# cy-rae/fast-slam

Hardware: AMD Instinct MI355X
Metric: particle-updates/s (higher is better)
Workload: dtype f64

## Files before the change

fast-slam_amd/csrc/fs2_api.hip:

```cpp
#include <hip/hip_runtime.h>

#include <sched.h>
#include <unistd.h>

#include <algorithm>
#include <atomic>
#include <chrono>
#include <condition_variable>
#include <functional>
#include <cmath>
#include <cstdarg>
#include <cstdio>
#include <cstdlib>
#include <cstring>
#include <mutex>
#include <string>
#include <thread>
#include <tuple>
#include <vector>

#include "../../include/fs2.h"
#include "fs2_comm.hpp"
#include "fs2_frontend.hpp"
#include "fs2_kernels.hpp"
// ... 280 lines not shown
struct MtCtx {
    fs2_mt_state in;
    double sigma = 0.0;
    int64_t N = 0, P = 0, A = 0, amb_cap = 0, pos0 = 0, have = 0, total = 0;
    int h0 = 0;
    fs2_mt_state *after = nullptr, *after_u0 = nullptr;
    double *u0_out = nullptr;
};

struct fs2_handle {
    fs2_config cfg{};
    int64_t n_global = 0, n = 0, first = 0;
    hipStream_t stream = nullptr;
    int cur = 0;
    double *x[2] = {}, *y[2] = {}, *yaw[2] = {}, *w[2] = {};
    int32_t *cnt[2] = {};
    char *pool = nullptr;
    int64_t npool = 0;
    GrowMem pool_vm, rpool_vm;
    GrowMem mark_vm, freel_vm, rmark_vm, rfreel_vm;
    int64_t bcnt_cap = 0, rbcnt_cap = 0;
    Desc *pt[2] = {};
    uint32_t *bbox[2] = {};
    XDesc *rdesc = nullptr;
    XDesc *udesc = nullptr;
    size_t udesc_cap = 0;
    unsigned long long *xt_key = nullptr;
    uint32_t *xt_ref = nullptr, *xt_uidx = nullptr, *xt_cmask = nullptr, *xt_cbase = nullptr;
    uint32_t *xt_eslot = nullptr, *xt_ulist = nullptr;
    int64_t xt_cap = 0, xt_ecap = 0;
    SumFrame frame{-127.0f, 1.0f, 1.0f};
    float ext_seen = 0.0f;
    float *slb = nullptr;
    float *slb_pass = nullptr;
    uint32_t *ext_dev = nullptr;
    size_t rdesc_cap = 0;
    int rows = 0;
    uint32_t *freel = nullptr;
    int64_t nfree = 0, cursor = 0;
    uint8_t *mark = nullptr;
    uint32_t *sent_mask = nullptr;
    uint8_t epoch = 0;
    int64_t *bcnt = nullptr;
    int64_t *nfree_dev = nullptr;
    uint64_t collections = 0;
    char *rpool = nullptr;
// ... 137 lines not shown
    std::vector<uint8_t> imported;
    PeerMaps peers_host{};
    PeerMaps *peers_dev = nullptr;
    uint8_t *ep_dev = nullptr, *epochs_dev = nullptr;
    int64_t remote_rows = 0;
    int64_t remote_pages = INT64_MAX;
    int64_t remote_bound() const { return std::min(remote_rows, remote_pages); }
    int32_t collect_next = 0;
    ChainSummary *dch_send = nullptr, *dch_recv = nullptr;
    RankRecordX *recx = nullptr, *recxs = nullptr;
    double *est_base = nullptr;
    int32_t *uop = nullptr;
    NpTailPlan *np_tail_g = nullptr;
    std::vector<std::pair<hipEvent_t, hipEvent_t>> xev;
    size_t xev_used = 0;
    struct Guard {
        char *at;
        const char *name;
    };
    std::vector<Guard> guards;

    MapRef map() const {
        return MapRef{pool, pt[cur], std::max<int64_t>(n, 1), rows, rpool, frame, slb, row_boxes(cur),
                      refs_shared ? peers_dev : nullptr};
    }
    uint32_t *row_boxes(int b) const { return rows <= kBBoxRows ? bbox[b] : nullptr; }
    int64_t nblocks() const { return (n + kBlock - 1) / kBlock; }
    int reduce() const {
        const int mode = cfg.reduce_mode;
        if (tp) {
            if (mode == FS2_REDUCE_SEQUENTIAL) return FS2_REDUCE_SEQUENTIAL;
            return (mode != FS2_REDUCE_PARALLEL && xsh_ok) ? FS2_REDUCE_EXACT : FS2_REDUCE_PARALLEL;
        }
        if (mode != FS2_REDUCE_AUTO) return mode;
        return n_global <= 4096 ? FS2_REDUCE_SEQUENTIAL : FS2_REDUCE_EXACT;
    }
    ChainParams chain(const double *a, const double *bsum, double *c, double *total, bool lazy) const {
        ChainParams p{};
        p.a = a;
        p.n = n;
        p.bsum = bsum;
        p.nb = (int32_t)nblocks();
        p.lazy = lazy ? 1 : 0;
        p.uinfo = uinfo;
        p.udelta = udelta;
        p.ugl = ugl;
        p.uol = uol;
        p.bD = bD;
        p.bC = bC;
// ... 43 lines not shown
        if (bytes <= cap) continue;
        hipFree(p);
        p = nullptr;
        cap = 0;
        HIP_TRY(h, hipMalloc(&p, bytes));
        cap = bytes;
    }
    return FS2_OK;
}

static int reserve_xfer_table(fs2_handle *h, int64_t cap, int64_t nrows, bool in_scan);
static int xfer_bufs(fs2_handle *h) {
    const int64_t S = std::max<int64_t>(h->n, 1) * h->rows;
    int lg = 10;
    while ((int64_t(1) << lg) < 2 * S && lg < 31) ++lg;
    const int rc = reserve_xfer_table(h, int64_t(1) << lg, S, false);
    return rc ? rc : recv_bufs(h, sizeof(XDesc) * (size_t)S);
}

static int sync_sets(fs2_handle *h) {
    if (!h->sets_dev) return FS2_OK;
    BufSet b[2];
    for (int k = 0; k < 2; ++k)
        b[k] = BufSet{h->x[k], h->y[k], h->yaw[k], h->w[k], h->cnt[k], h->pt[k], h->row_boxes(k)};
    HIP_TRY(h, copy_sync(h, h->sets_dev, b, sizeof b, hipMemcpyHostToDevice));
    return FS2_OK;
}

static int grow_rows(fs2_handle *h, int need_slots) {
    if (need_slots <= h->cap) return FS2_OK;
    if (need_slots > h->max_cap)
        return set_err(&h->err, FS2_ERR_CAPACITY, "map needs %d landmark slots, limit is %d",
                       need_slots, h->max_cap);
    int rows = (need_slots + kPageSlots - 1) / kPageSlots;
    if (h->rows > 0) {
        const int geo = h->rows + std::max(h->rows / 4, 8);
        const int lim = std::min(h->max_cap / kPageSlots, rows <= kBBoxRows ? kBBoxRows : INT_MAX);
        rows = std::max(rows, std::min(geo, lim));
    }
    const size_t row_bytes = sizeof(Desc) * (size_t)std::max<int64_t>(h->n, 1);
    HIP_TRY(h, hipStreamSynchronize(h->stream));
    for (int b = 0; b < 2; ++b) {
        Desc *p = nullptr;
        HIP_TRY(h, hipMalloc(&p, row_bytes * rows));
        if (h->pt[b] && b == h->cur) HIP_TRY(h, copy_sync(h, p, h->pt[b], row_bytes * h->rows, hipMemcpyDeviceToDevice));
        hipFree(h->pt[b]);
        h->pt[b] = p;
    }
    h->rows = rows;
    h->cap = rows * kPageSlots;
    if (int rc = sync_sets(h)) return rc;
    if (h->rdesc) return xfer_bufs(h);
    return FS2_OK;
}

static int refs_short(fs2_handle *h, const char *what) {
    return set_err(&h->err, FS2_ERR_CAPACITY,
                   "page_refs mode: the %s pool ran short between collective collections (pools shared with "
                   "the other ranks cannot grow; size them with page_pool / record_pool)",
                   what);
}

static int collect_body(fs2_handle *h, bool records);
struct PoolTimer {
    fs2_handle *h;
    bool grow;
    std::chrono::steady_clock::time_point t0 = std::chrono::steady_clock::now();
    ~PoolTimer() {
        const double ms = std::chrono::duration<double, std::milli>(std::chrono::steady_clock::now() - t0).count();
        if (grow) {
// ... 790 lines not shown
    return g_last_error.c_str();
}

static void free_handle(fs2_handle *h) {
    if (!h) return;
    int prev_dev = -1;
    if (hipGetDevice(&prev_dev) != hipSuccess) prev_dev = -1;
    if (prev_dev != h->cfg.device) (void)hipSetDevice(h->cfg.device);
    if (h->stream) hipStreamSynchronize(h->stream);
    if (h->mt.dstream) hipStreamSynchronize(h->mt.dstream);
    const bool vmm = h->pool_vm.base || h->rpool_vm.base || h->freel_vm.base || h->mark_vm.base ||
                     h->rfreel_vm.base || h->rmark_vm.base;
    if (vmm) hipDeviceSynchronize();
    if (h->refs_shared && h->tp && !h->tp->in_process()) {
        std::string e;
        if (h->tp->allgather(h->ep_dev, h->epochs_dev, 1, h->stream, &e) == FS2_OK) hipStreamSynchronize(h->stream);
        h->tp->unshare();
        if (h->tp->allgather(h->ep_dev, h->epochs_dev, 1, h->stream, &e) == FS2_OK) hipStreamSynchronize(h->stream);
    }
    for (int s = 0; s < 2; ++s) {
        hipFree(h->x[s]); hipFree(h->y[s]); hipFree(h->yaw[s]); hipFree(h->w[s]); hipFree(h->cnt[s]);
        hipFree(h->pt[s]);
        hipFree(h->bbox[s]);
    }
    hipFree(h->rdesc); hipFree(h->udesc);
    hipFree(h->xt_key); hipFree(h->xt_ref); hipFree(h->xt_uidx); hipFree(h->xt_cmask); hipFree(h->xt_cbase);
    hipFree(h->xt_eslot); hipFree(h->xt_ulist);
    hipFree(h->sent_mask);
    if (h->pool_vm.base) gm_free(h->pool_vm);
    else hipFree(h->pool);
    if (h->rpool_vm.base) gm_free(h->rpool_vm);
    else hipFree(h->rpool);
    if (h->freel_vm.base) gm_free(h->freel_vm); else hipFree(h->freel);
    if (h->mark_vm.base) gm_free(h->mark_vm); else hipFree(h->mark);
    if (h->rfreel_vm.base) gm_free(h->rfreel_vm); else hipFree(h->rfreel);
    if (h->rmark_vm.base) gm_free(h->rmark_vm); else hipFree(h->rmark);
    if (vmm) hipDeviceSynchronize();
    hipFree(h->bcnt); hipFree(h->nfree_dev);
    hipFree(h->rbcnt); hipFree(h->rnfree_dev);
    hipFree(h->slb); hipFree(h->slb_pass); hipFree(h->ext_dev);
    hipFree(h->rank_d); hipFree(h->rank_e); hipFree(h->iblk);
    hipFree(h->mlo); hipFree(h->mhi); hipFree(h->out_src); hipFree(h->runs); hipFree(h->runs_n);
    hipFree(h->rec); hipFree(h->recs); hipFree(h->totals); hipFree(h->xrow); hipFree(h->xmat);
    hipFree(h->sarena);
    hipFree(h->rarena);
    hipFree(h->cand); hipFree(h->ncand);
// ... 355 lines not shown

static int fold_profile(fs2_handle *h) {
    const int used = h->ev.used;
    h->ev.used = 0;
    for (int k = 0; k < used; ++k) {
        const int rc = fold_one(h, k);
        if (rc) return rc;
    }
    return FS2_OK;
}

static int fold_one(fs2_handle *h, int set) {
    const ProfScan &p = h->ev.scan[set];
    hipEvent_t *E = h->ev.e[set];
    HIP_TRY(h, hipEventSynchronize(E[3]));
    const DevStats &st = p.st;
    float a = 0, f = 0, r = 0, x = 0, t = 0;
    HIP_TRY(h, hipEventElapsedTime(&a, E[0], E[2]));
    HIP_TRY(h, hipEventElapsedTime(&r, E[5], E[3]));
    HIP_TRY(h, hipEventElapsedTime(&t, E[0], E[3]));
    const uint64_t n = (uint64_t)h->n, nblk = (uint64_t)h->nblocks();
    const uint64_t box_rows = h->row_boxes(h->cur) ? (uint64_t)h->rows : 0ull;
    const bool filt = h->cfg.gate_filter != 0;
    const uint64_t cand_bytes = filt ? sizeof(Desc) * st.groups + 128ull * st.opened + 8ull * st.words +
                                           8ull * n * p.passes + 4ull * box_rows * nblk
                                     : 0ull;
    const uint64_t upd_fixed = p.fixed_bytes + (filt ? 4ull * n * p.passes : 0ull) + 8ull * n * (uint64_t)p.m;
    const uint64_t exact_bytes = upd_fixed + (filt ? 8ull * st.words : 0ull) + 48ull * st.candidates +
                                 (64ull + sizeof(Desc)) * st.written + (2ull * kPageBytes + sizeof(Desc)) * st.cow_pages +
                                 8ull * box_rows * nblk;
    if (filt && p.m <= kMaxM) {
        HIP_TRY(h, hipEventElapsedTime(&f, E[0], E[1]));
        HIP_TRY(h, hipEventElapsedTime(&x, E[4], E[2]));
        h->prof.exact_launches += 1;
        h->prof.exact_ms += x;
        h->prof.filter_launches += 1;
        h->prof.filter_ms += f;
        h->prof.filter_bytes += cand_bytes;
        h->prof.model_groups += st.groups;
        h->prof.model_opened += st.opened;
        h->prof.model_words += st.words;
        h->prof.model_candidates += st.candidates;
        h->prof.model_written += st.written;
        h->prof.model_cow += st.cow_pages;
        h->prof.model_fixed_bytes += upd_fixed;
        h->prof.model_box_bytes += 12ull * box_rows * nblk;
    }
    h->prof.scans += 1;
    h->prof.update_launches += p.passes;
    h->prof.update_ms += a;
    h->prof.reduce_ms += r;
    h->prof.scan_ms += t;
    h->prof.update_bytes += cand_bytes + exact_bytes;
    if (st.resampled)
        h->prof.resample_bytes += 2ull * sizeof(Desc) * (st.resample_slots / kPageSlots) +
                                  2ull * 36ull * (uint64_t)h->n + 40ull * (uint64_t)h->n;
    return FS2_OK;
}

static int wait_flag(fs2_handle *h, unsigned long long seq) {
    const auto t0 = std::chrono::steady_clock::now();
    for (unsigned it = 0;; ++it) {
        if (__atomic_load_n(h->pub_flag, __ATOMIC_ACQUIRE) == seq) return FS2_OK;
        if ((it & 1023u) == 1023u && std::chrono::steady_clock::now() - t0 > std::chrono::milliseconds(50)) break;
        __builtin_ia32_pause();
    }
    HIP_TRY(h, hipStreamSynchronize(h->stream));
    if (__atomic_load_n(h->pub_flag, __ATOMIC_ACQUIRE) != seq)
        return set_err(&h->err, FS2_ERR_HIP, "scan statistics were not published");
// ... 54 lines not shown

    const int nxt = 1 - cur;
    ResampleParams rs{};
    rs.n = h->n;
    rs.N = h->n_global;
    rs.a = h->first;
    rs.ao = h->first;
    rs.keep = h->shard;
    rs.ranges_mode = (sh && h->follow) ? 1 : 3;
    rs.w = h->w[cur];
    rs.c = h->cbuf;
    rs.bsum = h->bsum;
    rs.nblk = (int32_t)((h->n + 1023) / 1024);
    rs.mlo = h->mlo;
    rs.mhi = h->mhi;
    rs.out_src = h->out_src;
    rs.runs = h->runs;
    rs.runs_n = h->runs_n;
    rs.x = h->x[cur]; rs.y = h->y[cur]; rs.yaw = h->yaw[cur]; rs.cnt = h->cnt[cur];
    rs.ox = h->x[nxt]; rs.oy = h->y[nxt]; rs.oyaw = h->yaw[nxt]; rs.ow = h->w[nxt]; rs.ocnt = h->cnt[nxt];
    rs.map = h->map();
    rs.opt = h->pt[nxt];
    rs.obbox = h->row_boxes(nxt);
    rs.rank_d = h->rank_d;
    rs.rank_e = h->rank_e;
    rs.iblk = h->iblk;
    rs.part_best_w = h->part_best_w;
    rs.part_best_i = h->part_best_i;
    rs.part_slots = h->part_slots;
    rs.stats = h->stats_dev;
    rs.rec = h->rec;
    rs.flip_margin = flip_margin;
    rs.use_chain = exact ? 1 : 0;
    rs.refs = h->refs ? 1 : 0;
    if (h->refs && h->xt_key) {
        rs.tkey = h->xt_key;
        rs.tcap = h->xt_cap;
        rs.tepoch = ++h->loc_epoch;
    }
    rs.chain = ChainView{h->uinfo, h->ugl, h->uol, h->bpd, h->bpc, h->seql, h->sout, h->uel, h->bpe};
    rs.gen = sh ? nullptr : h->gen_dev;

    const bool xsh = sh && exact;
    if (prof && exact && !xsh && h->n <= 0) HIP_TRY(h, hipEventRecord(E[5], s));
    if (exact && !xsh) {
        ChainParams cp = h->chain(h->w[cur], h->wpart, nullptr, &h->stats_dev->total, false);
// ... 79 lines not shown
            HIP_TRY(h, launch_chain_fold(h->dch_recv, G, h->shard, h->rank_of, nullptr, &h->stats_dev->offset,
                                         h->stats_dev, s));
            cp.chain_first = h->shard == 0 ? 1 : 0;
            cp.force_list0 = 1;
            cp.s_entry = &h->stats_dev->offset;
            HIP_TRY(h, launch_chain_walk_from(cp, s));
        }
        if (!sh) {
            rs.est_early = 1;
            rs.go = h->go_dev;
            rs.go_seq = pseq;
        }
        HIP_TRY(h, launch_resample_ranges(rs, s, sh));
        if (!sh)
            HIP_TRY(h, launch_tail_single(rs, rp, h->pub_stats_dev, h->pub_flag_dev, pseq, s, nullptr));
        if (sh) {
            rc = exchange_particles(h, rs);
            if (rc) return rc;
            if (posted_stats(h).max_count > h->cap) scan_alloc(h, "scan_alloc rows (slots M)", (size_t)posted_stats(h).max_count << 20);
            rc = grow_rows(h, posted_stats(h).max_count);
            if (rc) return rc;
            rs.opt = h->pt[nxt];
            rs.obbox = h->row_boxes(nxt);
            rc = reserve_recs(h, h->u_recv * kPageSlots, &rs.alloc);
            if (rc) return rc;
            rc = reserve_pages(h, h->u_recv, &rs.alloc);
            if (rc) return rc;
            rs.map = h->map();
            const size_t rbytes = sizeof(XDesc) * (size_t)std::max<int64_t>((int64_t)h->n_recv * h->rows, 1);
            const size_t ubytes = sizeof(XDesc) * (size_t)std::max<int64_t>(h->u_recv, 1);
            if (rbytes > h->rdesc_cap || ubytes > h->udesc_cap) {
                scan_alloc(h, "scan_alloc recv rows (MiB)", std::max(rbytes, ubytes));
                rc = recv_bufs(h, std::max(rbytes, ubytes));
                if (rc) return rc;
            }
            rs.udesc = h->udesc;
            rs.rdesc = h->rdesc;
        }
        HIP_TRY(h, launch_resample_apply(rs, sh, s));
        if (sh) {
            {
                CommTimer ct(h);
                rc = h->tp->allgather(h->rec, h->recs, sizeof(RankRecord), s, &h->err);
            }
            if (rc) return rc;
            HIP_TRY(h, launch_global_best(rp, s));
// ... 1633 lines not shown
```

fast-slam_amd/csrc/fs2_kernels.hpp:

```cpp
#pragma once

#include <hip/hip_ext.h>
#include <hip/hip_runtime.h>
#include <stdint.h>

#include <vector>

namespace fs2 {

constexpr int kBlock = 256;
constexpr int kPageSlots = 8;
constexpr int kMaxSlots = 4096;
constexpr int kMaxRows = kMaxSlots / kPageSlots;
constexpr int kMaxM = 4;
constexpr int kScanGroup = kPageSlots;
constexpr int kMaxCand = 8;

constexpr int kPageBytes = 128;
constexpr int kRecBytes = 48;
constexpr uint32_t kOwned = 0x80000000u;
constexpr uint32_t kIdMask = 0x7fffffffu;
constexpr uint32_t kRecIdLimit = 0xffffffffu;
typedef uint32_t Desc;
typedef uint2 XDesc;

struct SumFrame {
    float org, cell;
    float icell;
};
constexpr uint32_t kSumOpen = 0xff00ff00u;

constexpr int kBBoxRows = 256;
constexpr uint32_t kBoxEmpty = 0x00ff00ffu;

enum : int {
    kCWords, kCGroups, kCVisited, kCOpened, kCCandidates, kCWritten, kCAmbiguous, kCAppends, kCHits, kCCow, kCNew,
    kCRefVisits, kCSingular, kNumCounters
};

constexpr int64_t kWaveFill = 4096;
constexpr int64_t kFillChunk = 4096;
constexpr int kMaxLongRuns = 65536;
constexpr unsigned kTailFill = 64;

struct DevStats {
    double total;
    double sumsq;
    double n_eff;
    double u0;
    double best_w;
    double pose[3];
    int64_t best_index;
    int32_t resampled;
    int32_t max_count;
    int32_t error_flags;
    uint32_t pad1;
// ... 172 lines not shown
    float fe[kMaxM];
};

constexpr int kRefShift = 27;
constexpr uint32_t kRefIdMask = (1u << kRefShift) - 1u;
constexpr int kRefMaxRanks = 15;
struct PeerMaps {
    char *pool[kMaxRanks];
    char *recs[kMaxRanks];
    uint8_t *mark[kMaxRanks];
};
__host__ __device__ inline uint32_t ref_tag(uint32_t e) { return (e & 0x80000000u) ? 0u : (e >> kRefShift) & 15u; }
__host__ __device__ inline uint32_t ref_id(uint32_t e) { return (e & 0x80000000u) ? (e & 0x7fffffffu) : (e & kRefIdMask); }

struct MapRef {
    char *pool;
    Desc *pt;
    int64_t n;
    int32_t rows;
    char *recs;
    SumFrame frame;
    float *slb;
    uint32_t *bbox;
    const PeerMaps *peers;
};

struct PageAlloc {
    const uint32_t *freel;
    int64_t base;
    const uint32_t *rfreel;
    int64_t rbase;
};

struct BufSet {
    double *x, *y, *yaw, *w;
    int32_t *cnt;
    Desc *pt;
    uint32_t *bbox;
};

struct UpdateParams {
    int64_t n;
    int64_t blk0, blk1;
    int64_t nblk;
    int64_t gidx0;
    double *x, *y, *yaw, *w;
    int32_t *cnt;
    MapRef map;
    const double *noise;
    uint64_t seed, scan;
    double sigma;
    double rotation, translation;
    int32_t do_move;
    int32_t move_cand;
    int32_t m;
    int32_t k0;
    int32_t last_pass;
    double gate2;
    float gate2f;
    int32_t filter;
    PageAlloc alloc;
// ... 76 lines not shown
    double *w;
    double *c;
    double *bsum;
    int32_t nblk;
    int32_t lazy;
    uint32_t *gen;
    unsigned long long *tkey;
    int64_t tcap;
    uint32_t tepoch;
    double flip_margin;
    int32_t use_chain;
    ChainView chain;
    int32_t *mlo, *mhi;
    int32_t *out_src;
    int4 *runs;
    uint32_t *runs_n;
    const double *x, *y, *yaw;
    const int32_t *cnt;
    double *ox, *oy, *oyaw, *ow;
    int32_t *ocnt;
    MapRef map;
    Desc *opt;
    uint32_t *obbox;
    XDesc *rdesc;
    XDesc *udesc;
    PageAlloc alloc;
    int32_t *rank_d;
    int32_t *rank_e;
    int64_t *iblk;
    double *part_best_w;
    int64_t *part_best_i;
    unsigned long long *part_slots;
    DevStats *stats;
    RankRecord *rec;
    int32_t world, rank;
    PackPlan *plan;
    int64_t *xrow;
    char *sbuf[kMaxRanks];
    XferTable xt;
    uint32_t *sent_mask;
    double init_cov[4];
    int32_t npeers;
    RecvPeer peers[kMaxRanks];
    int32_t refs;
    int32_t est_early;
    unsigned long long *go;
// ... 196 lines not shown
```

fast-slam_amd/csrc/fs2_reduce.hpp:

```cpp
#pragma once

#include "fs2_device.hpp"
#include "fs2_kernels.hpp"

namespace fs2 {

#ifdef FS2_PHASE_TIMING
static __device__ unsigned long long g_tail[32];
#define FS2_TAIL_READER(name)                                                                \
    hipError_t name(unsigned long long out[32], int reset) {                                 \
        hipError_t e = hipMemcpyFromSymbol(out, HIP_SYMBOL(g_tail), sizeof(unsigned long long) * 32); \
        if (e == hipSuccess && reset) {                                                      \
            unsigned long long z[32] = {};                                                   \
            e = hipMemcpyToSymbol(HIP_SYMBOL(g_tail), z, sizeof z);                          \
        }                                                                                    \
        return e;                                                                            \
    }
#define FS2_TS_DECL unsigned long long ts_last_ = 0
#define FS2_TS(base, k)                                                                      \
    do {                                                                                     \
        if (blockIdx.x == 0 && threadIdx.x == 0) {                                           \
            const unsigned long long t_ = __builtin_amdgcn_s_memrealtime();                  \
            if ((k) > 0) atomicAdd(&g_tail[(base) + (k) - 1], t_ - ts_last_);               \
            ts_last_ = t_;                                                                   \
// ... 401 lines not shown
struct BoxLds {
    uint32_t lo[kBBoxRows], hi[kBBoxRows];
};
__device__ __forceinline__ void lds_box_set(BoxLds &s, int r, uint32_t b) {
    s.lo[r] = b & kBoxHalf;
    s.hi[r] = (b >> 8) & kBoxHalf;
}
__device__ __forceinline__ uint32_t lds_box_get(const BoxLds &s, int r) { return s.lo[r] | (s.hi[r] << 8); }
__device__ __forceinline__ void lds_box_merge(BoxLds &s, int r, uint32_t b) {
    const uint32_t blo = b & kBoxHalf, bhi = (b >> 8) & kBoxHalf;
    uint32_t lo = s.lo[r], hi = s.hi[r];
    for (uint32_t want = pk_min_u16(lo, blo); want != lo; want = pk_min_u16(lo, blo)) {
        const uint32_t prev = atomicCAS(&s.lo[r], lo, want);
        if (prev == lo) break;
        lo = prev;
    }
    for (uint32_t want = pk_max_u16(hi, bhi); want != hi; want = pk_max_u16(hi, bhi)) {
        const uint32_t prev = atomicCAS(&s.hi[r], hi, want);
        if (prev == hi) break;
        hi = prev;
    }
}

template <int MAXM>
__device__ __forceinline__ unsigned box_open_mask(uint32_t s, const uint32_t (&bc)[MAXM], int m) {
    const uint32_t xl = s & 0xffu, xh = (s >> 8) & 0xffu, yl = (s >> 16) & 0xffu, yh = s >> 24;
    unsigned om = 0u;
#pragma unroll
    for (int k = 0; k < MAXM; ++k)
        if (k < m && xl <= (bc[k] & 0xffu) && xh >= ((bc[k] >> 8) & 0xffu) && yl <= ((bc[k] >> 16) & 0xffu) &&
            yh >= (bc[k] >> 24))
            om |= 1u << k;
    return om;
}

__device__ __forceinline__ bool page_reject(uint32_t sum, const SumFrame &f, float slb, float fx, float fy,
                                            float fe, float gate2f) {
    const float xmin = sum_lo_val(f, sum & 0xffu), xmax = sum_hi_val(f, (sum >> 8) & 0xffu);
    const float ymin = sum_lo_val(f, (sum >> 16) & 0xffu), ymax = sum_hi_val(f, sum >> 24);
    const float Dx = fmaxf(fmaxf(xmin - fx, fx - xmax), 0.0f);
    const float Dy = fmaxf(fmaxf(ymin - fy, fy - ymax), 0.0f);
    const float Cx = fmaxf(fabsf(xmin), fabsf(xmax)) * 2.3841858e-7f;
    const float Cy = fmaxf(fabsf(ymin), fabsf(ymax)) * 2.3841858e-7f;
    const float lx = fmaxf(fmaf(Dx, 0.99999976f, -(fe + Cx)), 0.0f);
    const float ly = fmaxf(fmaf(Dy, 0.99999976f, -(fe + Cy)), 0.0f);
    return slb * fmaf(lx, lx, ly * ly) > gate2f;
// ... 42 lines not shown
```

fast-slam_amd/csrc/fs2_resample.hip:

```cpp
#include "fs2_chain.hpp"
#include "fs2_plan.hpp"

namespace fs2 {

constexpr int kScanPer = 4;
constexpr int kScanBlock = kBlock * kScanPer;


__global__ void k_global_total(const ReduceParams P) {
    double t = 0.0;
    for (int q = 0; q < P.world; ++q) {
        if (q == P.shard && P.est_base) *P.est_base = t;
        t = (q == 0) ? P.totals[P.rank_of[0]] : t + P.totals[P.rank_of[q]];
    }
    P.stats->total = t;
}

hipError_t launch_global_total(const ReduceParams &p, hipStream_t s) {
    hipLaunchKernelGGL(k_global_total, dim3(1), dim3(1), 0, s, p);
    return hipGetLastError();
}

__device__ double pairwise_sq(const double *a, int64_t n) {
    if (n < 8) {
// ... 1416 lines not shown
            nsb += s_wc[w];
        }
        if (first) s_sb[off + __popcll(fm & ((1ull << lane) - 1ull))] = s_src[t];
    }
    if (P.refs) {
        const unsigned long long br = block_sum_u64<kBlock>(nremote, lds_u);
        if (threadIdx.x == 0 && br) atomicAdd(&P.stats->remote_rows, br);
        __syncthreads();
        const unsigned long long bp = block_sum_u64<kBlock>(npages, lds_u);
        if (threadIdx.x == 0 && bp) atomicAdd(&P.stats->remote_pages, bp);
        __syncthreads();
    }
    const unsigned long long bs = block_sum_u64<kBlock>(slots, lds_u);
    block_argmax<kBlock>(bv, bi, lds_d, lds_l);
    if (threadIdx.x == 0) {
        P.part_best_w[blockIdx.x] = bv;
        P.part_best_i[blockIdx.x] = bi;
        P.part_slots[blockIdx.x] = bs;
    }
    if (bb && (int)threadIdx.x < P.map.rows) {
        uint32_t b = lds_box_get(s_bb, threadIdx.x);
        for (int q = 0; q < nsb; ++q) b = box_union(b, P.map.bbox[(int64_t)s_sb[q] * kBBoxRows + threadIdx.x]);
        P.obbox[(int64_t)blockIdx.x * kBBoxRows + threadIdx.x] = b;
    }
}

__global__ __launch_bounds__(kBlock) void k_bbox_build(const MapRef map, const int32_t *cnt, int64_t n) {
    __shared__ BoxLds s_bb;
    const int64_t i = (int64_t)blockIdx.x * kBlock + threadIdx.x;
    lds_box_set(s_bb, threadIdx.x, kBoxEmpty);
    const int c = (i < n) ? cnt[i] : 0;
    const int rows = (c + kPageSlots - 1) / kPageSlots;
    __syncthreads();
    const int wrows = wave_max_i(rows);
    for (int r = 0; r < wrows; ++r) {
        uint32_t b = kBoxEmpty;
        if (r < rows) {
            const float4 *mir = reinterpret_cast<const float4 *>(page_ptr_any(map, *pt_entry(map, r, i)));
            b = page_box(mir, min(kPageSlots, c - r * kPageSlots), map.frame);
        }
        b = wave_box_union(b);
        if ((threadIdx.x & 63) == 0) lds_box_merge(s_bb, r, b);
    }
    __syncthreads();
    if ((int)threadIdx.x < map.rows) map.bbox[(int64_t)blockIdx.x * kBBoxRows + threadIdx.x] = lds_box_get(s_bb, threadIdx.x);
}

hipError_t launch_bbox_build(MapRef map, const int32_t *cnt, hipStream_t s) {
    if (!map.bbox) return hipSuccess;
    const unsigned g = (unsigned)((map.n + kBlock - 1) / kBlock);
    hipLaunchKernelGGL(k_bbox_build, dim3(g), dim3(kBlock), 0, s, map, cnt, map.n);
    return hipGetLastError();
}

__device__ void estimate_body(const ResampleParams &P, int32_t nparts) {
    __shared__ double lds_d[16];
    __shared__ int64_t lds_l[16];
    __shared__ unsigned long long lds_u[16];
    double bv = -INFINITY;
    int64_t bi = INT64_MAX;
    unsigned long long sl = 0;
    for (int k = threadIdx.x; k < nparts; k += 1024) {
        argmax_combine(bv, bi, P.part_best_w[k], P.part_best_i[k]);
        sl += P.part_slots[k];
    }
    block_argmax<1024>(bv, bi, lds_d, lds_l);
    sl = block_sum_u64<1024>(sl, lds_u);
    if (threadIdx.x == 0) {
// ... 83 lines not shown
```

fast-slam_amd/csrc/fs2_update.hip:

```cpp
#include "fs2_chain.hpp"

namespace fs2 {

#ifdef FS2_PHASE_TIMING
__device__ unsigned long long g_phase[8];
#define FS2_PHASE(k)                                                                         \
    do {                                                                                     \
        const unsigned long long t_ = __builtin_amdgcn_s_memtime();                           \
        if ((threadIdx.x & 63) == 0 && (k) > 0) atomicAdd(&g_phase[(k) - 1], t_ - ph_last);   \
        ph_last = t_;                                                                        \
    } while (0)
#else
#define FS2_PHASE(k) do { } while (0)
#endif

constexpr int kDescAhead = 2;
constexpr int kCopyBatch = 8;

static_assert(kMaxCand == 8, "sort8 sorts the candidate list");

__device__ __forceinline__ uint64_t cand_entry(int slot, int pos, uint32_t rec) {
    return ((uint64_t)slot << 44) | ((uint64_t)pos << 32) | (uint64_t)rec;
}
__device__ __forceinline__ int cand_slot(uint64_t e) { return (int)(e >> 44); }
// ... 30 lines not shown
    py += ntr * sin(pyaw);
}

template <int MAXM>
__global__ __launch_bounds__(kBlock) void k_candidates(const UpdateParams P) {
    if (P.stats->error_flags & 8) return;
    __shared__ uint64_t s_list[kMaxCand][kBlock];
    __shared__ Band s_band[MAXM];
    __shared__ uint16_t s_rows[kBBoxRows];
    __shared__ uint8_t s_rmask[kBBoxRows];
    __shared__ int s_wc[kBlock / 64];
    const int tid = threadIdx.x;
    const int64_t n = P.n;
    const int64_t blk = P.blk0 + blockIdx.x;
    const int64_t i = blk * kBlock + tid;
    const bool live = i < n;
    MapRef map = P.map;
    const int32_t *cntp = P.cnt;
    double *xp = P.x, *yp = P.y, *yawp = P.yaw;
    if (P.gen) {
        const BufSet &b = P.sets[__builtin_amdgcn_readfirstlane(*(volatile const uint32_t *)P.gen) & 1u];
        map.pt = b.pt;
        map.bbox = b.bbox;
        cntp = b.cnt;
        xp = b.x;
        yp = b.y;
        yawp = b.yaw;
    }
    const int c = live ? cntp[i] : 0;
    if (P.move_cand && live) {
        double px = xp[i], py = yp[i], pyaw = yawp[i];
        move_particle(P, i, px, py, pyaw);
        xp[i] = px;
        yp[i] = py;
        yawp[i] = pyaw;
    }
    const Desc *ptrow = map.pt + (live ? i : 0);
    const float slb = *map.slb;
    if (blockIdx.x == 0 && tid == 0 && P.slb_pass) *P.slb_pass = slb;
    const int rlast = map.rows - 1;
    if (tid < MAXM) {
        Band b = band_none();
#pragma unroll
        for (int k = 0; k < MAXM; ++k)
            if (tid == k && k < P.m)
                b = gate_band(P.meas.fx[k], P.meas.fy[k], P.meas.fe[k], slb, P.gate2f, map.frame);
// ... 33 lines not shown
                    } else {
                        int mq = 0;
                        uint64_t me = s_list[0][tid];
#pragma unroll 1
                        for (int q = 1; q < kMaxCand; ++q) {
                            const uint64_t x = s_list[q][tid];
                            if (x > me) {
                                me = x;
                                mq = q;
                            }
                        }
                        if (e < me) s_list[mq][tid] = e;
                    }
                    ++nc;
                }
            }
        }
    };
    const bool use_bb = map.bbox != nullptr;
    int nrows = map.rows;
    if (use_bb) {
        unsigned rm = 0u;
        if (tid < map.rows) rm = box_open_mask<MAXM>(map.bbox[blk * kBBoxRows + tid], bc, P.m);
        const bool pass = rm != 0u;
        const uint64_t bm = __ballot(pass);
        const int wid = tid >> 6, lane = tid & 63;
        if (lane == 0) s_wc[wid] = __popcll(bm);
        __syncthreads();
        int off = 0;
        nrows = 0;
#pragma unroll
        for (int w = 0; w < kBlock / 64; ++w) {
            off += (w < wid) ? s_wc[w] : 0;
            nrows += s_wc[w];
        }
        if (pass) {
            const int at = off + __popcll(bm & ((1ull << lane) - 1ull));
            s_rows[at] = (uint16_t)tid;
            s_rmask[at] = (uint8_t)rm;
        }
        __syncthreads();
    }
    auto row_at = [&](int q) -> int { return use_bb ? (q < nrows ? (int)s_rows[q] : 0) : min(q, rlast); };
    Desc dq[kDescAhead];
#pragma unroll
    for (int q = 0; q < kDescAhead; ++q) dq[q] = ptrow[(int64_t)row_at(q) * n];
// ... 34 lines not shown
static __device__ __forceinline__ uint32_t sel_u32(int t, const uint32_t (&a)[K]) {
    uint32_t v = 0;
#pragma unroll
    for (int q = 0; q < K; ++q)
        if (t == q) v = a[q];
    return v;
}

template <int MAXM>
__global__ __launch_bounds__(kBlock) void k_update(const UpdateParams P) {
    if (P.stats->error_flags & 8) return;
    __shared__ Meas s_ms[MAXM];
    __shared__ double s_lik[MAXM][kBlock];
    __shared__ int16_t s_idx[MAXM][kBlock];
    union WaveScratch {
        uint2 cow[64 * (MAXM + 1)];
        struct {
            int best[MAXM][64], bpos[MAXM][64];
        } ov;
    };
    __shared__ WaveScratch s_ws[kBlock / 64];
    __shared__ float4 s_mv[MAXM][kBlock];
    __shared__ BoxLds s_bb;

#ifdef FS2_PHASE_TIMING
    unsigned long long ph_last = 0;
#endif
    const int tid = threadIdx.x;
    const int64_t blk = P.blk0 + blockIdx.x;
    const int64_t i = blk * kBlock + tid;
    const bool live = i < P.n;
    const int64_t n = P.n;
    if (tid < MAXM) s_ms[tid] = Meas{P.meas.d[tid], P.meas.b[tid], P.meas.ox[tid], P.meas.oy[tid]};
#pragma unroll
    for (int k = 0; k < MAXM; ++k) s_idx[k][tid] = (int16_t)-2;
    MapRef map = P.map;
    double *xp = P.x, *yp = P.y, *yawp = P.yaw, *wp = P.w;
    int32_t *cntp = P.cnt;
    if (P.gen) {
        const BufSet &b = P.sets[__builtin_amdgcn_readfirstlane(*(volatile const uint32_t *)P.gen) & 1u];
        xp = b.x;
        yp = b.y;
        yawp = b.yaw;
        wp = b.w;
        cntp = b.cnt;
        map.pt = b.pt;
        map.bbox = b.bbox;
    }
    if (map.bbox && tid < map.rows) lds_box_set(s_bb, tid, map.bbox[blk * kBBoxRows + tid]);
    __syncthreads();

    double px = 0.0, py = 0.0, pyaw = 0.0, w = 0.0;
    int c = 0;
    if (live) {
        px = xp[i];
        py = yp[i];
        pyaw = yawp[i];
        w = wp[i];
        c = cntp[i];
    }
    const int64_t il = live ? i : 0;
    int nalloc = 0;
    int nrec = 0;
    unsigned cow = 0, fresh = 0;
    float smin_w = INFINITY;
    uint64_t mods = 0;
    int nmod = 0;
    uint32_t frec[MAXM];
#pragma unroll
    for (int t = 0; t < MAXM; ++t) {
        frec[t] = (live && t < P.m) ? P.alloc.rfreel[P.alloc.rbase + (int64_t)t * n + i] : 0u;
    }
    FS2_PHASE(0);
#ifdef FS2_AB_NO_MOVE
    if (false) {
#else
    if (live && P.do_move && !P.move_cand) {
#endif
        move_particle(P, i, px, py, pyaw);
    }

    const M2 R{P.R[0], P.R[1], P.R[2], P.R[3]};
    auto box_note = [&](int row, uint32_t b) {
        if (map.bbox) lds_box_merge(s_bb, row, b);
    };
    unsigned pend = live ? ((1u << P.m) - 1u) : 0u;
    unsigned visited = 0, candidates = 0, written = 0, amb = 0, appends = 0;
    bool singular = false;
    const double gate2 = P.gate2;

    FS2_PHASE(1);
    int ncl = 0;
    bool overflow = false;
    if (live && P.filter) {
        const int nc = P.ncand[i];
        ncl = min(nc, kMaxCand);
        overflow = nc > kMaxCand;
    }

    auto visit = [&](int slot, int pos, Slot s) {
        ++candidates;
        bool mod = false;
        M2 I;
        bool ok = inv2(s.P, I);
        singular |= !ok;
        unsigned todo = ok ? pend : 0u;
        while (todo) {
// ... 244 lines not shown
            for (int u = 0; u < CB; ++u) {
                *reinterpret_cast<v4i *>(page_ptr(map.pool, d[u]) + off) = v[u];
            }
        };
        for (int base = 0; base < T; base += 8 * CB) {
            load_batch(base, va, da);
            store_batch(va, da);
        }
        __threadfence_block();
    }

    FS2_PHASE(3);
    {
#pragma unroll
        for (int t = 0; t < MAXM; ++t) {
            if (t < nmod) {
                const int j = (int)((mods >> (16 * t)) & 0xffffu);
                uint32_t id = 0;
#pragma unroll
                for (int u = 0; u < NR; ++u)
                    if (u == canon[t]) id = rdesc[u];
                const float4 m = s_mv[t][tid];
                reinterpret_cast<float4 *>(page_ptr(map.pool, id))[j & (kPageSlots - 1)] = m;
                box_note(rrow[t], point_box(m, map.frame));
            }
        }
        nrec = nmod;
#pragma unroll
        for (int t = 0; t < MAXM; ++t)
            if (t < nmod && canon[t] == t && ((cowm >> t) & 1u)) *pt_entry(map, rrow[t], il) = rdesc[t];
    }

    FS2_PHASE(4);
    int nap = 0;
    int arow = -1;
    Desc ad = 0u;
    bool ad_new = false;
    if (pend != 0u && c % kPageSlots != 0) {
        arow = c / kPageSlots;
#pragma unroll
        for (int u = 0; u < NR; ++u)
            if (u == canon[nmod]) {
                ad = rdesc[u];
                ad_new = (cowm >> u) & 1u;
            }
    }
    auto page_at = [&](int j) -> char * {
// ... 7 lines not shown
        for (int a = 0; a < nap; ++a) {
            const Slot s = load_slot(map, page_at(c + a), c + a);
            ++candidates;
            M2 I;
            if (!inv2(s.P, I)) {
                singular = true;
                break;
            }
            const double q = quad(I, mk.ox - s.mx, mk.oy - s.my);
            amb += ambiguous(q, gate2);
            if (q >= 0.0 && q < gate2) {
                hit = a;
                break;
            }
        }
        if (hit >= 0) {
            const int jh = c + hit;
            char *pg = page_at(jh);
            const uint32_t r = mirror_rec(load_mirror(pg, jh));
            Slot s = load_rec(map.recs, r);
            s_lik[k][tid] = ekf_update(s, px, py, pyaw, mk, R, singular);
            const float4 mv = store_slot(map, pg, jh, s, r, jh);
            smin_w = fminf(smin_w, mirror_s(mv) > 0.0f ? mirror_s(mv) : INFINITY);
            box_note(jh / kPageSlots, point_box(mv, map.frame));
            s_idx[k][tid] = (int16_t)(c + hit);
        } else {
            const Slot s{px + mk.d * cos(pyaw + mk.b), py + mk.d * sin(pyaw + mk.b),
                         M2{P.init_cov[0], P.init_cov[1], P.init_cov[2], P.init_cov[3]}};
            const int ja = c + nap;
            const uint32_t r = sel_u32(nrec, frec);
            ++nrec;
            if (ja % kPageSlots == 0) {
                if (arow >= 0 && ad_new) *pt_entry(map, arow, il) = ad;
                const uint32_t id = take_page(P.alloc, map.n, il, nalloc);
                arow = ja / kPageSlots;
                const float4 mv = store_slot(map, page_ptr(map.pool, id), ja, s, r, ja);
                smin_w = fminf(smin_w, mirror_s(mv) > 0.0f ? mirror_s(mv) : INFINITY);
                box_note(arow, point_box(mv, map.frame));
                ad = id | kOwned;
                ad_new = true;
                ++fresh;
            } else {
                const float4 mv = store_slot(map, page_ptr(map.pool, ad), ja, s, r, ja);
                smin_w = fminf(smin_w, mirror_s(mv) > 0.0f ? mirror_s(mv) : INFINITY);
                box_note(arow, point_box(mv, map.frame));
            }
            s_idx[k][tid] = (int16_t)-1;
            ++nap;
            ++appends;
        }
        ++written;
    }
    if (arow >= 0 && ad_new) *pt_entry(map, arow, il) = ad;
    c += nap;

    FS2_PHASE(5);
    unsigned hits = 0, refv = 0, napp = 0;
#pragma unroll
    for (int k = 0; k < MAXM; ++k) {
        const int ix = s_idx[k][tid];
        if (ix >= 0) {
            w *= s_lik[k][tid];
            ++hits;
            refv += (unsigned)ix + 1u;
        } else if (ix == -1) {
            refv += (unsigned)(c - nap + napp);
            ++napp;
        }
        if (live && P.assoc && k < P.m) P.assoc[(int64_t)(P.k0 + k) * n + i] = ix;
    }

    if (live) {
        if (P.do_move && !P.move_cand) {
            xp[i] = px;
            yp[i] = py;
            yawp[i] = pyaw;
        }
        wp[i] = w;
        cntp[i] = c;
    }

    FS2_PHASE(6);
    const unsigned cv[kNumCounters] = {0u, 0u, visited, 0u, candidates, written, amb, appends, hits, cow, fresh,
                                       refv, singular ? 1u : 0u};
    const unsigned assign =
        P.k0 != 0 ? 0u
                  : (P.filter ? ~((1u << kCWords) | (1u << kCGroups) | (1u << kCVisited) | (1u << kCOpened))
                              : 0xffffffffu);
    block_counters<kBlock, 0, kNumCounters>(cv, P.cpart, P.nblk, blk, assign, live ? w : 0.0,
                                            P.last_pass ? P.wpart + blk : nullptr);
    if (map.bbox && tid < map.rows) map.bbox[blk * kBBoxRows + tid] = lds_box_get(s_bb, tid);
    lower_slb(map.slb, smin_w);
}

hipError_t launch_candidates(const UpdateParams &p, hipStream_t s, hipEvent_t e0, hipEvent_t e1) {
    const unsigned grid = (unsigned)(p.blk1 - p.blk0);
    if (grid == 0 || !p.filter) return hipSuccess;
    FS2_LAUNCH_EV(k_candidates<kMaxM>, dim3(grid), dim3(kBlock), s, e0, e1, p);
    return hipGetLastError();
}

hipError_t launch_update(const UpdateParams &p, hipStream_t s, hipEvent_t e0, hipEvent_t e1) {
    const unsigned grid = (unsigned)(p.blk1 - p.blk0);
    if (grid == 0) return hipSuccess;
    FS2_LAUNCH_EV(k_update<kMaxM>, dim3(grid), dim3(kBlock), s, e0, e1, p);
    return hipGetLastError();
}

template <int MAXM, int PHASE>
__global__ __launch_bounds__(kBlock) void k_localize(const LocalizeParams P) {
    __shared__ Band s_band[MAXM];
    __shared__ uint16_t s_rows[kBBoxRows];
    __shared__ int s_wc[kBlock / 64];
    __shared__ unsigned long long s_base;
// ... 578 lines not shown
```

Baseline: 463.1 million.

## Add per-slot-position bounding boxes to tighten candidate gating per block

Result: slower. 390.0 million (-15.8%).

```diff
diff --git a/fast-slam_amd/csrc/fs2_api.hip b/fast-slam_amd/csrc/fs2_api.hip
--- a/fast-slam_amd/csrc/fs2_api.hip
+++ b/fast-slam_amd/csrc/fs2_api.hip
@@ -326,6 +326,7 @@
     int64_t bcnt_cap = 0, rbcnt_cap = 0;
     Desc *pt[2] = {};
     uint32_t *bbox[2] = {};
+    uint32_t *sbox[2] = {};
     XDesc *rdesc = nullptr;
     XDesc *udesc = nullptr;
     size_t udesc_cap = 0;
@@ -509,9 +510,10 @@
 
     MapRef map() const {
         return MapRef{pool, pt[cur], std::max<int64_t>(n, 1), rows, rpool, frame, slb, row_boxes(cur),
-                      refs_shared ? peers_dev : nullptr};
+                      slot_boxes(cur), refs_shared ? peers_dev : nullptr};
     }
     uint32_t *row_boxes(int b) const { return rows <= kBBoxRows ? bbox[b] : nullptr; }
+    uint32_t *slot_boxes(int b) const { return rows <= kBBoxRows ? sbox[b] : nullptr; }
     int64_t nblocks() const { return (n + kBlock - 1) / kBlock; }
     int reduce() const {
         const int mode = cfg.reduce_mode;
@@ -601,7 +603,8 @@
     if (!h->sets_dev) return FS2_OK;
     BufSet b[2];
     for (int k = 0; k < 2; ++k)
-        b[k] = BufSet{h->x[k], h->y[k], h->yaw[k], h->w[k], h->cnt[k], h->pt[k], h->row_boxes(k)};
+        b[k] = BufSet{h->x[k], h->y[k], h->yaw[k], h->w[k], h->cnt[k], h->pt[k], h->row_boxes(k),
+                      h->slot_boxes(k)};
     HIP_TRY(h, copy_sync(h, h->sets_dev, b, sizeof b, hipMemcpyHostToDevice));
     return FS2_OK;
 }
@@ -625,6 +628,20 @@
         if (h->pt[b] && b == h->cur) HIP_TRY(h, copy_sync(h, p, h->pt[b], row_bytes * h->rows, hipMemcpyDeviceToDevice));
         hipFree(h->pt[b]);
         h->pt[b] = p;
+    }
+    for (int b = 0; b < 2; ++b) {
+        uint32_t *p = nullptr;
+        if (rows <= kBBoxRows) {
+            const size_t nb = (size_t)std::max<int64_t>(h->nblocks(), 1), wg = sizeof(uint32_t) * kPageSlots;
+            HIP_TRY(h, hipMalloc(&p, nb * rows * wg));
+            HIP_TRY(h, hipMemsetD32Async((hipDeviceptr_t)p, (int)kBoxEmpty, nb * rows * kPageSlots, h->stream));
+            if (h->sbox[b] && b == h->cur && h->rows > 0)
+                HIP_TRY(h, hipMemcpy2DAsync(p, rows * wg, h->sbox[b], h->rows * wg, h->rows * wg, nb,
+                                            hipMemcpyDeviceToDevice, h->stream));
+            HIP_TRY(h, hipStreamSynchronize(h->stream));
+        }
+        hipFree(h->sbox[b]);
+        h->sbox[b] = p;
     }
     h->rows = rows;
     h->cap = rows * kPageSlots;
@@ -1461,6 +1478,7 @@
         hipFree(h->x[s]); hipFree(h->y[s]); hipFree(h->yaw[s]); hipFree(h->w[s]); hipFree(h->cnt[s]);
         hipFree(h->pt[s]);
         hipFree(h->bbox[s]);
+        hipFree(h->sbox[s]);
     }
     hipFree(h->rdesc); hipFree(h->udesc);
     hipFree(h->xt_key); hipFree(h->xt_ref); hipFree(h->xt_uidx); hipFree(h->xt_cmask); hipFree(h->xt_cbase);
@@ -1862,13 +1880,14 @@
     const uint64_t n = (uint64_t)h->n, nblk = (uint64_t)h->nblocks();
     const uint64_t box_rows = h->row_boxes(h->cur) ? (uint64_t)h->rows : 0ull;
     const bool filt = h->cfg.gate_filter != 0;
+    const uint64_t slot_box_bytes = 4ull * kPageSlots * box_rows * nblk * p.passes;
     const uint64_t cand_bytes = filt ? sizeof(Desc) * st.groups + 128ull * st.opened + 8ull * st.words +
-                                           8ull * n * p.passes + 4ull * box_rows * nblk
+                                           8ull * n * p.passes + 4ull * box_rows * nblk + slot_box_bytes
                                      : 0ull;
     const uint64_t upd_fixed = p.fixed_bytes + (filt ? 4ull * n * p.passes : 0ull) + 8ull * n * (uint64_t)p.m;
     const uint64_t exact_bytes = upd_fixed + (filt ? 8ull * st.words : 0ull) + 48ull * st.candidates +
                                  (64ull + sizeof(Desc)) * st.written + (2ull * kPageBytes + sizeof(Desc)) * st.cow_pages +
-                                 8ull * box_rows * nblk;
+                                 8ull * box_rows * nblk + slot_box_bytes;
     if (filt && p.m <= kMaxM) {
         HIP_TRY(h, hipEventElapsedTime(&f, E[0], E[1]));
         HIP_TRY(h, hipEventElapsedTime(&x, E[4], E[2]));
@@ -1884,7 +1903,7 @@
         h->prof.model_written += st.written;
         h->prof.model_cow += st.cow_pages;
         h->prof.model_fixed_bytes += upd_fixed;
-        h->prof.model_box_bytes += 12ull * box_rows * nblk;
+        h->prof.model_box_bytes += 12ull * box_rows * nblk + 2ull * slot_box_bytes;
     }
     h->prof.scans += 1;
     h->prof.update_launches += p.passes;
@@ -1985,6 +2004,7 @@
     rs.map = h->map();
     rs.opt = h->pt[nxt];
     rs.obbox = h->row_boxes(nxt);
+    rs.osbox = h->slot_boxes(nxt);
     rs.rank_d = h->rank_d;
     rs.rank_e = h->rank_e;
     rs.iblk = h->iblk;
@@ -2110,6 +2130,7 @@
             if (rc) return rc;
             rs.opt = h->pt[nxt];
             rs.obbox = h->row_boxes(nxt);
+            rs.osbox = h->slot_boxes(nxt);
             rc = reserve_recs(h, h->u_recv * kPageSlots, &rs.alloc);
             if (rc) return rc;
             rc = reserve_pages(h, h->u_recv, &rs.alloc);
diff --git a/fast-slam_amd/csrc/fs2_kernels.hpp b/fast-slam_amd/csrc/fs2_kernels.hpp
--- a/fast-slam_amd/csrc/fs2_kernels.hpp
+++ b/fast-slam_amd/csrc/fs2_kernels.hpp
@@ -32,6 +32,7 @@
 
 constexpr int kBBoxRows = 256;
 constexpr uint32_t kBoxEmpty = 0x00ff00ffu;
+
 
 enum : int {
     kCWords, kCGroups, kCVisited, kCOpened, kCCandidates, kCWritten, kCAmbiguous, kCAppends, kCHits, kCCow, kCNew,
@@ -250,6 +251,7 @@
     SumFrame frame;
     float *slb;
     uint32_t *bbox;
+    uint32_t *sbox;
     const PeerMaps *peers;
 };
 
@@ -265,6 +267,7 @@
     int32_t *cnt;
     Desc *pt;
     uint32_t *bbox;
+    uint32_t *sbox;
 };
 
 struct UpdateParams {
@@ -387,6 +390,7 @@
     MapRef map;
     Desc *opt;
     uint32_t *obbox;
+    uint32_t *osbox;
     XDesc *rdesc;
     XDesc *udesc;
     PageAlloc alloc;
diff --git a/fast-slam_amd/csrc/fs2_reduce.hpp b/fast-slam_amd/csrc/fs2_reduce.hpp
--- a/fast-slam_amd/csrc/fs2_reduce.hpp
+++ b/fast-slam_amd/csrc/fs2_reduce.hpp
@@ -447,6 +447,28 @@
     }
 }
 
+__device__ __forceinline__ bool lds_sbox_merge(uint32_t *s, int e, uint32_t b) {
+    uint32_t cur = s[e];
+    bool grew = false;
+    for (uint32_t want = box_union(cur, b); want != cur; want = box_union(cur, b)) {
+        grew = true;
+        const uint32_t prev = atomicCAS(&s[e], cur, want);
+        if (prev == cur) break;
+        cur = prev;
+    }
+    return grew;
+}
+
+template <int MAXM>
+__device__ __forceinline__ unsigned box_open_mask(uint32_t s, const uint32_t (&bc)[MAXM], int m);
+template <int MAXM>
+__device__ __forceinline__ unsigned slot_boxes_open_mask(const uint32_t *sb, const uint32_t (&bc)[MAXM], int m) {
+    const uint4 a = reinterpret_cast<const uint4 *>(sb)[0], b = reinterpret_cast<const uint4 *>(sb)[1];
+    return box_open_mask<MAXM>(a.x, bc, m) | box_open_mask<MAXM>(a.y, bc, m) | box_open_mask<MAXM>(a.z, bc, m) |
+           box_open_mask<MAXM>(a.w, bc, m) | box_open_mask<MAXM>(b.x, bc, m) | box_open_mask<MAXM>(b.y, bc, m) |
+           box_open_mask<MAXM>(b.z, bc, m) | box_open_mask<MAXM>(b.w, bc, m);
+}
+
 template <int MAXM>
 __device__ __forceinline__ unsigned box_open_mask(uint32_t s, const uint32_t (&bc)[MAXM], int m) {
     const uint32_t xl = s & 0xffu, xh = (s >> 8) & 0xffu, yl = (s >> 16) & 0xffu, yh = s >> 24;
diff --git a/fast-slam_amd/csrc/fs2_resample.hip b/fast-slam_amd/csrc/fs2_resample.hip
--- a/fast-slam_amd/csrc/fs2_resample.hip
+++ b/fast-slam_amd/csrc/fs2_resample.hip
@@ -1462,28 +1462,74 @@
         uint32_t b = lds_box_get(s_bb, threadIdx.x);
         for (int q = 0; q < nsb; ++q) b = box_union(b, P.map.bbox[(int64_t)s_sb[q] * kBBoxRows + threadIdx.x]);
         P.obbox[(int64_t)blockIdx.x * kBBoxRows + threadIdx.x] = b;
+        if (P.osbox && P.map.sbox) {
+            uint32_t sb[kPageSlots];
+#pragma unroll
+            for (int u = 0; u < kPageSlots; ++u) sb[u] = recv ? b : kBoxEmpty;
+            for (int q = 0; q < nsb && !recv; ++q) {
+                const uint4 *src = reinterpret_cast<const uint4 *>(
+                    P.map.sbox + ((int64_t)s_sb[q] * P.map.rows + threadIdx.x) * kPageSlots);
+                const uint4 lo = src[0], hi = src[1];
+                sb[0] = box_union(sb[0], lo.x); sb[1] = box_union(sb[1], lo.y);
+                sb[2] = box_union(sb[2], lo.z); sb[3] = box_union(sb[3], lo.w);
+                sb[4] = box_union(sb[4], hi.x); sb[5] = box_union(sb[5], hi.y);
+                sb[6] = box_union(sb[6], hi.z); sb[7] = box_union(sb[7], hi.w);
+            }
+            uint4 *dst = reinterpret_cast<uint4 *>(P.osbox + ((int64_t)blockIdx.x * P.map.rows + threadIdx.x) * kPageSlots);
+            dst[0] = make_uint4(sb[0], sb[1], sb[2], sb[3]);
+            dst[1] = make_uint4(sb[4], sb[5], sb[6], sb[7]);
+        }
     }
 }
 
 __global__ __launch_bounds__(kBlock) void k_bbox_build(const MapRef map, const int32_t *cnt, int64_t n) {
     __shared__ BoxLds s_bb;
+    __shared__ uint32_t s_sb[kBBoxRows * kPageSlots];
     const int64_t i = (int64_t)blockIdx.x * kBlock + threadIdx.x;
     lds_box_set(s_bb, threadIdx.x, kBoxEmpty);
+    for (int e = threadIdx.x; e < kBBoxRows * kPageSlots; e += kBlock) s_sb[e] = kBoxEmpty;
     const int c = (i < n) ? cnt[i] : 0;
     const int rows = (c + kPageSlots - 1) / kPageSlots;
     __syncthreads();
     const int wrows = wave_max_i(rows);
     for (int r = 0; r < wrows; ++r) {
+        const float4 *mir = r < rows ? reinterpret_cast<const float4 *>(page_ptr_any(map, *pt_entry(map, r, i))) : nullptr;
+        const int lane = threadIdx.x & 63;
+        float x0 = INFINITY, x1 = -INFINITY, y0 = INFINITY, y1 = -INFINITY;
+        bool open = false, any = false;
+#pragma unroll
+        for (int u = 0; u < kPageSlots; ++u) {
+            const bool have = mir && r * kPageSlots + u < c;
+            const float4 mv = have ? mir[u] : make_float4(0.0f, 0.0f, 0.0f, 0.0f);
+            const bool ok = have && isfinite(mv.x) && isfinite(mv.y) && mirror_s(mv) > 0.0f;
+            auto fmin_ = [](float a, float b) { return fminf(a, b); };
+            auto fmax_ = [](float a, float b) { return fmaxf(a, b); };
+            const float wx0 = lane63(dpp_scan(ok ? mv.x : INFINITY, INFINITY, fmin_));
+            const float wx1 = lane63(dpp_scan(ok ? mv.x : -INFINITY, -INFINITY, fmax_));
+            const float wy0 = lane63(dpp_scan(ok ? mv.y : INFINITY, INFINITY, fmin_));
+            const float wy1 = lane63(dpp_scan(ok ? mv.y : -INFINITY, -INFINITY, fmax_));
+            const bool wopen = __ballot(have && !ok) != 0ull, wany = __ballot(ok) != 0ull;
+            if (lane == u) {
+                x0 = wx0; x1 = wx1; y0 = wy0; y1 = wy1;
+                open = wopen;
+                any = wany;
+            }
+        }
         uint32_t b = kBoxEmpty;
-        if (r < rows) {
-            const float4 *mir = reinterpret_cast<const float4 *>(page_ptr_any(map, *pt_entry(map, r, i)));
-            b = page_box(mir, min(kPageSlots, c - r * kPageSlots), map.frame);
-        }
+        if (open) b = kSumOpen;
+        else if (any)
+            b = sum_lo(map.frame, x0) | (sum_hi(map.frame, x1) << 8) | (sum_lo(map.frame, y0) << 16) |
+                (sum_hi(map.frame, y1) << 24);
+        if (map.sbox && lane < kPageSlots) lds_sbox_merge(s_sb, r * kPageSlots + lane, b);
         b = wave_box_union(b);
-        if ((threadIdx.x & 63) == 0) lds_box_merge(s_bb, r, b);
+        if (lane == 0) lds_box_merge(s_bb, r, b);
     }
     __syncthreads();
     if ((int)threadIdx.x < map.rows) map.bbox[(int64_t)blockIdx.x * kBBoxRows + threadIdx.x] = lds_box_get(s_bb, threadIdx.x);
+    if (map.sbox) {
+        uint32_t *sb = map.sbox + (int64_t)blockIdx.x * map.rows * kPageSlots;
+        for (int e = threadIdx.x; e < map.rows * kPageSlots; e += kBlock) sb[e] = s_sb[e];
+    }
 }
 
 hipError_t launch_bbox_build(MapRef map, const int32_t *cnt, hipStream_t s) {
diff --git a/fast-slam_amd/csrc/fs2_update.hip b/fast-slam_amd/csrc/fs2_update.hip
--- a/fast-slam_amd/csrc/fs2_update.hip
+++ b/fast-slam_amd/csrc/fs2_update.hip
@@ -76,6 +76,7 @@
         const BufSet &b = P.sets[__builtin_amdgcn_readfirstlane(*(volatile const uint32_t *)P.gen) & 1u];
         map.pt = b.pt;
         map.bbox = b.bbox;
+        map.sbox = b.sbox;
         cntp = b.cnt;
         xp = b.x;
         yp = b.y;
@@ -155,6 +156,8 @@
     if (use_bb) {
         unsigned rm = 0u;
         if (tid < map.rows) rm = box_open_mask<MAXM>(map.bbox[blk * kBBoxRows + tid], bc, P.m);
+        if (rm != 0u && map.sbox)
+            rm = slot_boxes_open_mask<MAXM>(map.sbox + (blk * map.rows + tid) * kPageSlots, bc, P.m);
         const bool pass = rm != 0u;
         const uint64_t bm = __ballot(pass);
         const int wid = tid >> 6, lane = tid & 63;
@@ -235,6 +238,8 @@
     __shared__ WaveScratch s_ws[kBlock / 64];
     __shared__ float4 s_mv[MAXM][kBlock];
     __shared__ BoxLds s_bb;
+    __shared__ uint32_t s_sb[kBBoxRows * kPageSlots];
+    __shared__ int s_sgrew;
 
 #ifdef FS2_PHASE_TIMING
     unsigned long long ph_last = 0;
@@ -259,8 +264,12 @@
         cntp = b.cnt;
         map.pt = b.pt;
         map.bbox = b.bbox;
+        map.sbox = b.sbox;
     }
     if (map.bbox && tid < map.rows) lds_box_set(s_bb, tid, map.bbox[blk * kBBoxRows + tid]);
+    if (map.sbox)
+        for (int e = tid; e < map.rows * kPageSlots; e += kBlock) s_sb[e] = map.sbox[blk * map.rows * kPageSlots + e];
+    if (tid == 0) s_sgrew = 0;
     __syncthreads();
 
     double px = 0.0, py = 0.0, pyaw = 0.0, w = 0.0;
@@ -294,8 +303,9 @@
     }
 
     const M2 R{P.R[0], P.R[1], P.R[2], P.R[3]};
-    auto box_note = [&](int row, uint32_t b) {
+    auto box_note = [&](int row, int pos, uint32_t b) {
         if (map.bbox) lds_box_merge(s_bb, row, b);
+        if (map.sbox && lds_sbox_merge(s_sb, row * kPageSlots + (pos & (kPageSlots - 1)), b)) s_sgrew = 1;
     };
     unsigned pend = live ? ((1u << P.m) - 1u) : 0u;
     unsigned visited = 0, candidates = 0, written = 0, amb = 0, appends = 0;
@@ -586,7 +596,7 @@
                     if (u == canon[t]) id = rdesc[u];
                 const float4 m = s_mv[t][tid];
                 reinterpret_cast<float4 *>(page_ptr(map.pool, id))[j & (kPageSlots - 1)] = m;
-                box_note(rrow[t], point_box(m, map.frame));
+                box_note(rrow[t], j, point_box(m, map.frame));
             }
         }
         nrec = nmod;
@@ -640,7 +650,7 @@
             s_lik[k][tid] = ekf_update(s, px, py, pyaw, mk, R, singular);
             const float4 mv = store_slot(map, pg, jh, s, r, jh);
             smin_w = fminf(smin_w, mirror_s(mv) > 0.0f ? mirror_s(mv) : INFINITY);
-            box_note(jh / kPageSlots, point_box(mv, map.frame));
+            box_note(jh / kPageSlots, jh, point_box(mv, map.frame));
             s_idx[k][tid] = (int16_t)(c + hit);
         } else {
             const Slot s{px + mk.d * cos(pyaw + mk.b), py + mk.d * sin(pyaw + mk.b),
@@ -654,14 +664,14 @@
                 arow = ja / kPageSlots;
                 const float4 mv = store_slot(map, page_ptr(map.pool, id), ja, s, r, ja);
                 smin_w = fminf(smin_w, mirror_s(mv) > 0.0f ? mirror_s(mv) : INFINITY);
-                box_note(arow, point_box(mv, map.frame));
+                box_note(arow, ja, point_box(mv, map.frame));
                 ad = id | kOwned;
                 ad_new = true;
                 ++fresh;
             } else {
                 const float4 mv = store_slot(map, page_ptr(map.pool, ad), ja, s, r, ja);
                 smin_w = fminf(smin_w, mirror_s(mv) > 0.0f ? mirror_s(mv) : INFINITY);
-                box_note(arow, point_box(mv, map.frame));
+                box_note(arow, ja, point_box(mv, map.frame));
             }
             s_idx[k][tid] = (int16_t)-1;
             ++nap;
@@ -708,6 +718,8 @@
     block_counters<kBlock, 0, kNumCounters>(cv, P.cpart, P.nblk, blk, assign, live ? w : 0.0,
                                             P.last_pass ? P.wpart + blk : nullptr);
     if (map.bbox && tid < map.rows) map.bbox[blk * kBBoxRows + tid] = lds_box_get(s_bb, tid);
+    if (map.sbox && s_sgrew)
+        for (int e = tid; e < map.rows * kPageSlots; e += kBlock) map.sbox[blk * map.rows * kPageSlots + e] = s_sb[e];
     lower_slb(map.slb, smin_w);
 }
 
```
